# urgent-challenge/urgent2026_challenge_track1

Hardware: AMD Instinct MI355X
Metric: utterances/sec (4 s @ 48 kHz) train step (higher is better)
Workload: dtype bf16

## Files before the change

### include/urse.h

```cpp
#ifndef URSE_H_
#define URSE_H_
#include <stdint.h>

#ifdef __cplusplus
extern "C" {
#endif

#define URSE_OK 0
#define URSE_ERR_INVALID_ARG (-1)
#define URSE_ERR_LAUNCH (-2)
#define URSE_ERR_UNSUPPORTED (-3)
#define URSE_ERR_RUNTIME (-4)

#define URSE_F32 0
#define URSE_BF16 1
#define URSE_F16 2
#define URSE_BF16_ACT_F16 3

#define URSE_WIN_RECT 0
#define URSE_WIN_HANN 1

int urse_version(void);
const char* urse_last_error(void);

#define URSE_KV_NT_BRES 0
#define URSE_KV_NT_RING 1
#define URSE_KV_NT_RING_WIDE 2
#define URSE_KV_NT_128 3
#define URSE_KV_NT_GROUPED_RING 4
#define URSE_KV_NT_GROUPED_128 5
#define URSE_KV_TN_RING 6
#define URSE_KV_TN_RING_T 7
#define URSE_KV_TN_DUAL 8
#define URSE_KV_TN_128 9
#define URSE_KV_TN_GROUPED 10
#define URSE_KV_LSTM_FWD_STREAM 11
#define URSE_KV_LSTM_FWD_WIDE 12
#define URSE_KV_LSTM_FWD_CLUSTER 13
#define URSE_KV_LSTM_FWD_CLUSTER2 14
#define URSE_KV_LSTM_BWD_STREAM16 15
#define URSE_KV_LSTM_BWD_STREAM32 16
#define URSE_KV_LSTM_BWD_CLUSTER 17
#define URSE_KV_LSTM_BWD_SPLIT 18
#define URSE_KV_STFT960 19
#define URSE_KV_STFT_GENERIC 20
#define URSE_KV_ISTFT_GENERIC 21
#define URSE_KV_ISTFT960 22
#define URSE_KV_LSTM_FWD_RW 23
#define URSE_KV_TN_ACT_F16 24
#define URSE_KV_LSTM_FWD_RWX 25
#define URSE_KV_LSTM_BWD_NSPLIT 26
#define URSE_KV_LSTM_FWD_CLUSTERX 27
#define URSE_KV_COUNT 32
int urse_launch_count(int variant);
int urse_launch_counts_reset(void);

int urse_stft_fwd(const float* wav, const int32_t* lens, float* spec, int B, int L, int n_fft, int hop,
                  int window, void* stream);
int urse_istft_fwd(const float* spec, float* wav, int B, int T, int n_fft, int hop, int L_out, int window,
                   void* stream);
int urse_istft_bwd(const float* grad_wav, float* grad_spec, int B, int T, int n_fft, int hop, int L_out,
                   int window, void* stream);

int urse_gemm_nt(const void* A, int64_t lda, const void* B, int64_t ldb, void* C, int64_t ldc, const float* bias,
                 const float* resid, int64_t ldr, int64_t M, int64_t N, int64_t K, int in_dtype, int out_dtype,
                 int act, void* stream);
int urse_gemm_nt_gnstats(const void* A, int64_t lda, const void* B, int64_t ldb, float* C, int64_t ldc, const float* bias,
                         const float* resid, int64_t ldr, int64_t M, int64_t N, int64_t K, int in_dtype, int act,
                         double* stats, int64_t rows_per_group, void* stream);
int urse_gemm_nt_gnbwd(const void* A, int64_t lda, const void* B, int64_t ldb, float* C, int64_t M, int64_t N, int64_t K, int in_dtype,
                       const float* x, const double* stats, const float* gamma, double* sums, float* dgamma, float* dbeta, float* part,
                       int slots, int64_t rows_per_group, float eps, void* stream);
int urse_gemm_nt_grouped(const void* descs, int groups, int max_blocks, int in_dtype, int out_dtype, int act,
                         void* stream);
int urse_gemm_nt_grouped_h(const void* descs, const int64_t* host_descs, int groups, int in_dtype, int out_dtype,
                           int act, void* stream);
int urse_gemm_tn(const void* A, int64_t lda, const void* B, int64_t ldb, float* C, int64_t ldc, float* colsum,
                 int64_t R, int64_t Mo, int64_t No, int64_t shift, int64_t inner, int64_t period,
                 int64_t invalid_step, int64_t perm_h, int dtype, int target_workgroups, void* stream);
int urse_gemm_tn_act_f16_supported(int64_t R, int64_t Mo, int64_t No, int64_t No2, int with_colsum, int64_t inner, int64_t period);
int urse_gemm_tn_dual(const void* A, int64_t lda, const void* B, int64_t ldb, float* C, int64_t ldc, float* colsum,
                      const void* B2, int64_t ldb2, float* C2, int64_t ldc2, int64_t R, int64_t Mo, int64_t No, int64_t No2,
                      int64_t shift, int64_t inner, int64_t period, int64_t invalid_step, int64_t perm_h, int dtype,
                      int target_workgroups, void* stream);
int urse_gemm_tn_grouped(const void* descs, int groups, int max_blocks, int dtype, void* stream);

int urse_groupnorm_fwd(const float* x, const float* gamma, const float* beta, const float* add, void* y, double* stats,
                       int B, int T, int Kg, int W, int N, int Np, int gstride, float eps, int out_dtype, void* y_bf16, void* stream);
int urse_groupnorm_stats(const float* x, double* stats, int B, int T, int Kg, int W, int N, void* stream);
int urse_groupnorm_apply(const float* x, const float* gamma, const float* beta, const float* add, void* y, const double* stats,
                         int B, int T, int Kg, int W, int N, int Np, int gstride, float eps, int out_dtype, void* y_bf16, void* stream);
int urse_groupnorm_bwd(const float* x, const float* dy, const double* stats, const float* gamma, const float* dres,
                       float* dx, float* dgamma, float* dbeta, double* sums, int B, int T, int Kg, int W, int N,
                       int gstride, float eps, void* dx_packed, int ldp, void* stream);
int urse_groupnorm_bwd_apply(const float* x, const float* dy, const double* stats, const double* sums, const float* gamma,
                             const float* dres, float* dx, int B, int T, int Kg, int W, int N, int gstride, float eps, void* dx_packed,
                             int ldp, void* stream);
int urse_pack2d(const void* in, int64_t ldi, int in_dtype, void* out, int64_t ldo, int out_dtype, int rows, int cols,
                int out_rows, int out_cols, int transpose, void* stream);

int urse_pack_segments(const float* in, void* out, const void* segs, int nseg, int blocks_per_seg, int transpose,
                       int out_dtype, void* stream);

int urse_lstm_pack(const float* wih, const float* whh, const float* bih, const float* bhh, void* wih_p, void* wihT_p,
                   float* bias, void* whh_frag, void* whhT_frag, int N, int Np, int H, int Hp, int dtype,
// ... 173 lines not shown
```

### urgent2026_challenge_track1_amd/csrc/gemm.hip

```cpp
#include <stdlib.h>

#include <type_traits>
#include "urse_common.h"

namespace urse {

typedef __bf16 bf16x8_t __attribute__((ext_vector_type(8)));
typedef short short8_t __attribute__((ext_vector_type(8)));
typedef short short4_t __attribute__((ext_vector_type(4)));
typedef float f32x4_t __attribute__((ext_vector_type(4)));

struct GemmDesc {
  const char* A;
  const char* B;
  char* C;
  const float* bias;
  const float* resid;
  long lda, ldb, ldc;
  long M, N, K;
  long ldr;
};

constexpr int BM = 128, BN = 128;
constexpr int SLAB = 64;
// ... 1142 lines not shown
#pragma unroll 1
    for (int h = 0; h < nh; ++h) {
      if constexpr (BH) compute_h(slot + h);
      else compute(slot + h);
      T2ST(4 + h);
    }
    slot ^= 2;
#ifdef T224STAMP
    ++it_;
#endif
  }
  }
  asm volatile("s_waitcnt vmcnt(0)" ::: "memory");

#pragma unroll
  for (int j = 0; j < NT; ++j) {
    const long v = n0 + (wn * NT + j) * 16 + (lane & 15);
    float* dst = nullptr;
    long ld = 0, col = 0;
    if (v < p.No) { dst = p.C; ld = p.ldc; col = v; }
    else if (v >= No8 && v < V) { dst = p.C2; ld = p.ldc2; col = v - No8; }
    else if (v == vones) { dst = p.colsum; ld = 1; col = 0; }
    if (dst == nullptr) continue;
#pragma unroll
    for (int i = 0; i < MT; ++i)
#pragma unroll
      for (int r = 0; r < 4; ++r) {
        const long row = m0 + wm * (MT * 16) + i * 16 + (lane >> 4) * 4 + r;
        atomicAdd(dst + tn_perm(row, p.perm_h) * ld + col, acc[i][j][r]);
      }
  }
}

static void launch_tn_dma(int ntw, int csm, dim3 grid, hipStream_t st, const TnArgs& p, int cvt = 0) {
  if (cvt == 1) { hipLaunchKernelGGL((gemm_tn_dma_kernel<7, 2, 1>), grid, dim3(512), 0, st, p); return; }
#define URSE_TN_L(N_, C_) hipLaunchKernelGGL((gemm_tn_dma_kernel<N_, C_>), grid, dim3(512), 0, st, p)
  if (ntw == 7) { if (csm == 0) URSE_TN_L(7, 0); else if (csm == 1) URSE_TN_L(7, 1); else URSE_TN_L(7, 2); }
  else { if (csm == 0) URSE_TN_L(8, 0); else if (csm == 1) URSE_TN_L(8, 1); else URSE_TN_L(8, 2); }
#undef URSE_TN_L
}

struct NtExtra {
  double* gstats;
  long rpg;
  const float* gnb_x;
  const double* gnb_stats;
  const float* gnb_gamma;
  double* gnb_sums;
  float* gnb_part;
  int gnb_slots;
  float gnb_eps;
};

template <typename TO, int NTW, int ACT, int BMX, int WNC, int GNB = 0, typename TI = bf16_t>
__device__ __forceinline__ void gemm_nt_dma_body(const GemmDesc& d, double* gstats = nullptr, long rpg = 0, const NtExtra* xt = nullptr) {
  constexpr int BNX = 16 * NTW * WNC, NWV = BMX / 64 * WNC, NTHR = NWV * 64;
  constexpr int BNR = WNC == 2 ? 256 : 16 * NTW * WNC;
  constexpr int NST = NWV == 8 ? URSE_NT_NST : 3, STAGE = (BMX + BNR) * 64, BOFF = BMX * 64;
  constexpr int AI = (BMX / 16 + NWV - 1) / NWV;
  constexpr int BI = (BNR / 16 + NWV - 1) / NWV;
  constexpr int DPW = AI + BI;
  static_assert(AI * NWV * 16 == BMX, "A image blocks divide evenly over the waves");
  __shared__ __attribute__((aligned(1024))) char lds[NST * STAGE + 1024];
  const int tn = (int)((d.N + BNX - 1) / BNX), tm = (int)((d.M + BMX - 1) / BMX);
  if ((int)blockIdx.x >= tm * tn) return;
  const int bid = xcd_remap(blockIdx.x, tm * tn);
  const int tile_m = bid / tn, tile_n = bid - tile_m * tn;
  const long m0 = (long)tile_m * BMX, n0 = (long)tile_n * BNX;
  const int tid = threadIdx.x, lane = tid & 63;
  const int w = __builtin_amdgcn_readfirstlane(tid >> 6), wm = w / WNC, wn = w % WNC;
  const int nk = (int)(d.K / 32);
  const char* zsrc = reinterpret_cast<const char*>(g_tn_zero_page) + lane * 16;
  const int srow = lane >> 2, schunk = (lane & 3) ^ ((lane >> 3) & 3);
  const int lc = lane & 15, lr = lane >> 4;
  const int foff = lc * 64 + ((lr ^ ((lc >> 1) & 3)) << 4);

  const char* pa[AI];
  const char* pb[BI];
  bool aok[AI], bok[BI];
#pragma unroll
  for (int j = 0; j < AI; ++j) {
    const int rowl = 16 * (AI * w + j) + srow;
    aok[j] = rowl < BMX && m0 + rowl < d.M;
    pa[j] = d.A + ((m0 + rowl) * d.lda) * 2 + schunk * 16;
  }
#pragma unroll
  for (int j = 0; j < BI; ++j) {
    const int rowl = 16 * (BI * w + j) + srow;
    bok[j] = rowl < BNX && n0 + rowl < d.N;
    pb[j] = d.B + ((n0 + rowl) * d.ldb) * 2 + schunk * 16;
  }
  auto issue = [&](int kt, int slot) {
    char* sbase = lds + slot * STAGE;
    const bool kin = kt < nk;
#pragma unroll
    for (int j = 0; j < AI; ++j) glds16((kin && aok[j]) ? pa[j] + (long)kt * 64 : zsrc, sbase + (AI * w + j) * 1024);
#pragma unroll
    for (int j = 0; j < BI; ++j) {
      const int blk = BI * w + j;
      glds16((kin && bok[j]) ? pb[j] + (long)kt * 64 : zsrc, blk < BNR / 16 ? sbase + BOFF + blk * 1024 : lds + NST * STAGE);
    }
  };
#pragma unroll
  for (int s = 0; s < NST - 1; ++s) issue(s, s);

  constexpr int OS = sizeof(TO);
  f32x4_t bv[NTW];
#pragma unroll
  for (int j = 0; j < NTW; ++j) {
    const long col = n0 + (wn * NTW + j) * 16 + lr * 4;
#pragma unroll
    for (int r = 0; r < 4; ++r) bv[j][r] = (d.bias && col + r < d.N) ? d.bias[col + r] : 0.f;
  }
  f32x4_t acc[4][NTW];
#pragma unroll
  for (int i = 0; i < 4; ++i)
#pragma unroll
    for (int j = 0; j < NTW; ++j) acc[i][j] = f32x4_t{0.f, 0.f, 0.f, 0.f};

  int slot = 0;
  for (int kt = 0; kt < nk; ++kt) {
    if ((NST - 2) * DPW == 12) asm volatile("s_waitcnt vmcnt(12)" ::: "memory");
    else if ((NST - 2) * DPW == 10) asm volatile("s_waitcnt vmcnt(10)" ::: "memory");
    else if ((NST - 2) * DPW == 8) asm volatile("s_waitcnt vmcnt(8)" ::: "memory");
    else asm volatile("s_waitcnt vmcnt(6)" ::: "memory");
    static_assert((NST - 2) * DPW == 12 || (NST - 2) * DPW == 10 || (NST - 2) * DPW == 8 || (NST - 2) * DPW == 6, "wait count");
    __builtin_amdgcn_s_barrier();
    int nslot = slot + NST - 1;
    if (nslot >= NST) nslot -= NST;
    issue(kt + NST - 1, nslot);
    const char* As = lds + slot * STAGE + wm * 4096 + foff;
    const char* Bs = lds + slot * STAGE + BOFF + wn * NTW * 1024 + foff;
    short8_t a[4];
#pragma unroll
    for (int i = 0; i < 4; ++i) a[i] = *reinterpret_cast<const short8_t*>(As + i * 1024);
    short8_t b[NTW];
#pragma unroll
    for (int j = 0; j < NTW; ++j) b[j] = *reinterpret_cast<const short8_t*>(Bs + j * 1024);
#if URSE_NT_SETPRIO
    __builtin_amdgcn_s_setprio(1);
#endif
#pragma unroll
    for (int j = 0; j < NTW; ++j)
#pragma unroll
      for (int i = 0; i < 4; ++i) acc[i][j] = Frag<TI>::mma(b[j], a[i], acc[i][j]);
#if URSE_NT_SETPRIO
    __builtin_amdgcn_s_setprio(0);
#endif
    if (++slot == NST) slot = 0;
  }
  asm volatile("s_waitcnt vmcnt(0)" ::: "memory");
  __syncthreads();
#ifdef NABL_NO_EPI
  if (acc[0][0][0] == 123.456f) d.C[0] = 1;
  return;
#endif

  constexpr int CP = BNX * OS + 16;
  constexpr int RPP = (BMX * CP <= NST * STAGE) ? BMX : ((BMX / 2 * CP <= NST * STAGE) ? BMX / 2 : BMX / 4);
  static_assert(RPP * CP <= NST * STAGE && RPP >= 64, "staging does not fit");
  constexpr int EPC = 16 / OS;
  constexpr int CPR = BNX / EPC;
  TO* C = reinterpret_cast<TO*>(d.C);
  constexpr bool C2K = __is_same(TI, f16_t) && OS == 2 && ACT == 1;
  bf16_t* C2 = (C2K && d.resid) ? reinterpret_cast<bf16_t*>(const_cast<float*>(d.resid)) : nullptr;
  const bool vec_ok = ((d.ldc * OS) % 16 == 0) && ((reinterpret_cast<uintptr_t>(d.C) % 16) == 0) &&
                      (!d.resid || ACT == 2 || (((d.ldr * 4) % 16 == 0) && (reinterpret_cast<uintptr_t>(d.resid) % 16) == 0)) &&
                      (!C2 || (d.ldr * 2) % 16 == 0);
  float gsa = 0.f, gqa = 0.f, gsb = 0.f, gqb = 0.f;
  const bool gst = OS == 4 && gstats != nullptr;
  const long gidx = gst ? m0 / rpg : 0, gbound = gst ? (gidx + 1) * rpg : 0;
  float gnb_m[2] = {0.f, 0.f}, gnb_r[2] = {0.f, 0.f}, gnb_ga[4] = {0.f, 0.f, 0.f, 0.f}, gnb_dg[4] = {0.f, 0.f, 0.f, 0.f}, gnb_db[4] = {0.f, 0.f, 0.f, 0.f};
  long gnb_g0 = 0, gnb_bound = 0;
  constexpr int GXI = GNB ? (RPP + NTHR / CPR - 1) / (NTHR / CPR) : 1, GXA = GXI < 8 ? GXI : 8;
  float4 gnb_xpre[GXI];
  if constexpr (GNB) {
    gnb_g0 = m0 / xt->rpg;
    gnb_bound = (gnb_g0 + 1) * xt->rpg;
    const double cnt = (double)xt->rpg * (double)d.N;
#pragma unroll
    for (int q = 0; q < 2; ++q) {
      const long g = gnb_g0 + q;
      if (g * xt->rpg < d.M) {
        const double mu = xt->gnb_stats[g * 2] / cnt;
        double var = xt->gnb_stats[g * 2 + 1] / cnt - mu * mu;
        if (var < 0.0) var = 0.0;
        gnb_m[q] = (float)mu;
        gnb_r[q] = (float)(1.0 / sqrt(var + (double)xt->gnb_eps));
      }
    }
    const int chf = tid % (BNX / (16 / OS));
    const long col = n0 + chf * (16 / OS);
#pragma unroll
    for (int q = 0; q < 4; ++q) gnb_ga[q] = (col + q < d.N) ? xt->gnb_gamma[col + q] : 0.f;
  }
#pragma unroll 1
  for (int pass = 0; pass < BMX / RPP; ++pass) {
    if (pass > 0) __syncthreads();
    if constexpr (GNB) {
      constexpr int SLOTS = NTHR / CPR, XI = (RPP + SLOTS - 1) / SLOTS;
      const int slot = tid / CPR, chf = tid - slot * CPR;
      const long col = n0 + chf * EPC;
      static_assert(XI == GXI, "prefetch array");
#pragma unroll
      for (int i = 0; i < GXA; ++i) {
        const int lr_ = slot + i * SLOTS;
        const long row = m0 + pass * RPP + lr_;
        const bool ok = slot < SLOTS && col < d.N && lr_ < RPP && row < d.M;
        gnb_xpre[i] = ok ? *reinterpret_cast<const float4*>(xt->gnb_x + row * d.ldc + col) : make_float4(0.f, 0.f, 0.f, 0.f);
      }
    }
    if ((wm * 64) / RPP == pass) {
      const int rbase = (wm * 64) % RPP;
// ... 145 lines not shown
      pb[tid] = make_float4(gnb_db[0], gnb_db[1], gnb_db[2], gnb_db[3]);
    }
    __syncthreads();
    if (tid < 4) {
      double t = 0.0;
      for (int i = 0; i < NWV; ++i) t += red[i * 4 + tid];
      const long g = gnb_g0 + (tid >> 1);
      if ((tid < 2 || gnb_bound < m0 + BMX) && g * xt->rpg < d.M) atomicAdd(xt->gnb_sums + g * 2 + (tid & 1), t);
    }
    if (tid >= 64 && tid < 64 + CPR) {
      const int chf = tid - 64;
      const long col = n0 + chf * EPC;
      if (col < d.N) {
        float4 sg = make_float4(0.f, 0.f, 0.f, 0.f), sb = sg;
        for (int i = 0; i < SLOTS; ++i) {
          const float4 a = pg[i * CPR + chf], bq = pb[i * CPR + chf];
          sg.x += a.x; sg.y += a.y; sg.z += a.z; sg.w += a.w;
          sb.x += bq.x; sb.y += bq.y; sb.z += bq.z; sb.w += bq.w;
        }
        float* part = xt->gnb_part + (long)(blockIdx.x % xt->gnb_slots) * 2 * d.N;
        const float vg[4] = {sg.x, sg.y, sg.z, sg.w}, vb[4] = {sb.x, sb.y, sb.z, sb.w};
        for (int q = 0; q < 4 && col + q < d.N; ++q) {
          atomicAdd(part + col + q, vg[q]);
          atomicAdd(part + d.N + col + q, vb[q]);
        }
      }
    }
    return;
  }
  if (gst) {
    __syncthreads();
    double* red = reinterpret_cast<double*>(lds);
    const double r0 = wave_sum_d((double)gsa), r1 = wave_sum_d((double)gqa), r2 = wave_sum_d((double)gsb), r3 = wave_sum_d((double)gqb);
    if (lane == 0) { red[w * 4] = r0; red[w * 4 + 1] = r1; red[w * 4 + 2] = r2; red[w * 4 + 3] = r3; }
    __syncthreads();
    if (tid < 4) {
      double t = 0.0;
      for (int i = 0; i < NWV; ++i) t += red[i * 4 + tid];
      const long g = gidx + (tid >> 1);
      if (tid < 2 || gbound < m0 + BMX) {
        if (g * rpg < d.M) atomicAdd(gstats + g * 2 + (tid & 1), t);
      }
    }
  }
}

template <typename TO, int NTW, int ACT, int BMX, int WNC = 2, typename TI = bf16_t>
__global__ void __launch_bounds__(BMX / 64 * WNC * 64) gemm_nt_dma_kernel(GemmDesc d, NtExtra x) {
  gemm_nt_dma_body<TO, NTW, ACT, BMX, WNC, 0, TI>(d, x.gstats, x.rpg);
}

__global__ void __launch_bounds__(512) gemm_nt_dma_gnb_kernel(GemmDesc d, NtExtra x) {
  gemm_nt_dma_body<float, 7, 0, 256, 2, 1>(d, nullptr, 0, &x);
}

__global__ void gnb_fold_kernel(const float* __restrict__ part, int slots, int N, float* __restrict__ dgamma, float* __restrict__ dbeta) {
  const int c = blockIdx.x * blockDim.x + threadIdx.x;
  if (c >= N) return;
  float a = 0.f, b = 0.f;
  for (int s = 0; s < slots; ++s) { a += part[(long)s * 2 * N + c]; b += part[(long)s * 2 * N + N + c]; }
  dgamma[c] += a;
  dbeta[c] += b;
}

template <typename TO, int ACT, typename TI = bf16_t>
__global__ void __launch_bounds__(512) gemm_nt_dma_grouped_kernel(const GemmDesc* __restrict__ descs) {
  const GemmDesc d = descs[blockIdx.y];
  gemm_nt_dma_body<TO, 7, ACT, 256, 2, 0, TI>(d);
}

template <int ACT, typename TI = bf16_t>
__global__ void __launch_bounds__(512) gemm_nt_bres_kernel(GemmDesc d, int wg_per_slice) {
  constexpr int BMX = 256, NTW = 7, BNX = 224, NST = 3, STAGE = BMX * 64, KSTEPS = 7, BRES = KSTEPS * 14 * 1024;
  __shared__ __attribute__((aligned(1024))) char lds[BRES + NST * STAGE];
  char* ring = lds + BRES;
  const int tm = (int)((d.M + BMX - 1) / BMX);
  const int tile_n = blockIdx.x / wg_per_slice, part = blockIdx.x - tile_n * wg_per_slice;
  const long n0 = (long)tile_n * BNX;
  const int tid = threadIdx.x, lane = tid & 63;
  const int w = __builtin_amdgcn_readfirstlane(tid >> 6), wm = w >> 1, wn = w & 1;
  const int nk = (int)(d.K / 32);
  const char* zsrc = reinterpret_cast<const char*>(g_tn_zero_page) + lane * 16;
  const int srow = lane >> 2, schunk = (lane & 3) ^ ((lane >> 3) & 3);
  const int lc = lane & 15, lr = lane >> 4;
  const int foff = lc * 64 + ((lr ^ ((lc >> 1) & 3)) << 4);
  for (int blk = w; blk < nk * 14; blk += 8) {
    const int kt = blk / 14, b = blk - kt * 14;
    const long row = n0 + b * 16 + srow;
    glds16(row < d.N ? d.B + (row * d.ldb) * 2 + schunk * 16 + (long)kt * 64 : zsrc, lds + blk * 1024);
  }
  f32x4_t bv[NTW];
#pragma unroll
  for (int j = 0; j < NTW; ++j) {
    const long col = n0 + (wn * NTW + j) * 16 + lr * 4;
#pragma unroll
    for (int r = 0; r < 4; ++r) bv[j][r] = (d.bias && col + r < d.N) ? d.bias[col + r] : 0.f;
  }
  bf16_t* C = reinterpret_cast<bf16_t*>(d.C);
  auto tile_src = [&](int mt, const char* (&pa)[2], bool (&aok)[2]) __attribute__((always_inline)) {
#pragma unroll
    for (int j = 0; j < 2; ++j) {
      const long row = (long)mt * BMX + 16 * (2 * w + j) + srow;
      aok[j] = mt < tm && row < d.M;
      pa[j] = d.A + (row * d.lda) * 2 + schunk * 16;
    }
  };
// ... 295 lines not shown
    long rpp = (M + parts - 1) / parts;
    rpp = (rpp + WR_ROWS - 1) / WR_ROWS * WR_ROWS;
    dim3 grid((unsigned)(tn * parts));
    hipStream_t st = (hipStream_t)stream;
    note_launch(URSE_KV_NT_BRES);
    if (act == 0) hipLaunchKernelGGL(gemm_nt_wreg_kernel<0>, grid, dim3(448), 0, st, d, parts, rpp);
    else hipLaunchKernelGGL(gemm_nt_wreg_kernel<1>, grid, dim3(448), 0, st, d, parts, rpp);
    URSE_CHECK_LAUNCH("urse_gemm_nt");
    return URSE_OK;
  }
#endif
  if (bres_mode && in16 && out16 && !no_dma && M >= 8192 && N >= g_nt_bres_min_n && K % 32 == 0 &&
      K >= 96 && K <= 224 && !resid && act != 2 && (ldc * 2) % 16 == 0 && ((uintptr_t)C % 16) == 0) {
    const int tn = (int)((N + 223) / 224);
    int per = g_nt_bres_wgs / tn;
    if (per < 1) per = 1;
    dim3 grid((unsigned)(tn * per));
    hipStream_t st = (hipStream_t)stream;
    note_launch(URSE_KV_NT_BRES);
    if (f16) {
      if (act == 0) hipLaunchKernelGGL((gemm_nt_bres_kernel<0, f16_t>), grid, dim3(512), 0, st, d, per);
      else hipLaunchKernelGGL((gemm_nt_bres_kernel<1, f16_t>), grid, dim3(512), 0, st, d, per);
    } else if (act == 0) hipLaunchKernelGGL(gemm_nt_bres_kernel<0>, grid, dim3(512), 0, st, d, per);
    else hipLaunchKernelGGL(gemm_nt_bres_kernel<1>, grid, dim3(512), 0, st, d, per);
    URSE_CHECK_LAUNCH("urse_gemm_nt");
    return URSE_OK;
  }
  if (in16 && !no_dma && M >= 2048 && N >= 160 && K % 32 == 0 && K >= 96 && !(f16 && act == 2)) {
    const long pad7 = (N + 223) / 224 * 224, pad8 = (N + 255) / 256 * 256;
    int ntw = pad7 <= pad8 ? 7 : 8;
    if (const char* e = getenv("URSE_NT_NTW")) ntw = atoi(e) == 8 ? 8 : 7;
    int bmx = 256;
    if (const char* e = getenv("URSE_NT_BMX")) bmx = atoi(e) == 128 ? 128 : 256;
    int wide = g_nt_wide_default && K <= g_nt_wide_maxk && N >= 1792 && out_dtype == URSE_BF16 && (N + 447) / 448 * 448 <= pad7 + 64;
    if (const char* e = getenv("URSE_NT_WIDE")) wide = atoi(e) != 0 && N >= 448;
    if (f16) { wide = 0; bmx = 256; }
    const long tl = wide ? ((M + 127) / 128) * ((N + 447) / 448) : ((M + bmx - 1) / bmx) * ((N + 32L * ntw - 1) / (32L * ntw));
    URSE_CHECK_ARG(tl < (1L << 31), "urse_gemm_nt: too many tiles");
    dim3 grid((unsigned)tl);
    hipStream_t st = (hipStream_t)stream;
    if (gstats && out_dtype == URSE_F32 && act != 2 && !wide && rpg >= bmx) {
      xtra.gstats = gstats;
      xtra.rpg = rpg;
      if (fused) *fused = 1;
    }
#define URSE_NT_DMA(TO_, NTW_, ACT_, BMX_) \
  hipLaunchKernelGGL((gemm_nt_dma_kernel<TO_, NTW_, ACT_, BMX_>), grid, dim3(BMX_ * 2), 0, st, d, xtra)
#define URSE_NT_DMA_W(TO_, ACT_) \
  hipLaunchKernelGGL((gemm_nt_dma_kernel<TO_, 7, ACT_, 128, 4>), grid, dim3(512), 0, st, d, xtra)
#define URSE_NT_DMA_B(TO_, NTW_, ACT_) do { if (wide) URSE_NT_DMA_W(TO_, ACT_); else if (bmx == 128) URSE_NT_DMA(TO_, NTW_, ACT_, 128); else URSE_NT_DMA(TO_, NTW_, ACT_, 256); } while (0)
#define URSE_NT_DMA_ACT(TO_, NTW_) \
  do { if (act == 0) URSE_NT_DMA_B(TO_, NTW_, 0); else if (act == 1) URSE_NT_DMA_B(TO_, NTW_, 1); else URSE_NT_DMA_B(TO_, NTW_, 2); } while (0)
    note_launch(wide ? URSE_KV_NT_RING_WIDE : URSE_KV_NT_RING);
    if (f16) {
#define URSE_NT_DMA_H(TO_, NTW_, ACT_) hipLaunchKernelGGL((gemm_nt_dma_kernel<TO_, NTW_, ACT_, 256, 2, f16_t>), grid, dim3(512), 0, st, d, xtra)
#define URSE_NT_DMA_H_ACT(TO_, NTW_) do { if (act == 0) URSE_NT_DMA_H(TO_, NTW_, 0); else URSE_NT_DMA_H(TO_, NTW_, 1); } while (0)
      if (out_dtype == URSE_F16) { if (ntw == 7) URSE_NT_DMA_H_ACT(f16_t, 7); else URSE_NT_DMA_H_ACT(f16_t, 8); }
      else { if (ntw == 7) URSE_NT_DMA_H_ACT(float, 7); else URSE_NT_DMA_H_ACT(float, 8); }
    } else if (out_dtype == URSE_BF16) {
      if (ntw == 7) URSE_NT_DMA_ACT(bf16_t, 7); else URSE_NT_DMA_ACT(bf16_t, 8);
    } else {
      if (ntw == 7) URSE_NT_DMA_ACT(float, 7); else URSE_NT_DMA_ACT(float, 8);
    }
    URSE_CHECK_LAUNCH("urse_gemm_nt");
    return URSE_OK;
  }
  const long blocks = ((M + BM - 1) / BM) * ((N + BN - 1) / BN);
  URSE_CHECK_ARG(blocks < (1L << 31), "urse_gemm_nt: too many tiles");
  note_launch(URSE_KV_NT_128);
  return dispatch_nt(nullptr, d, 1, (int)blocks, in_dtype, out_dtype, act, (hipStream_t)stream);
}

extern "C" int urse_gemm_nt(const void* A, int64_t lda, const void* B, int64_t ldb, void* C, int64_t ldc,
                            const float* bias, const float* resid, int64_t ldr, int64_t M, int64_t N, int64_t K,
                            int in_dtype, int out_dtype, int act, void* stream) {
  return gemm_nt_impl(A, lda, B, ldb, C, ldc, bias, resid, ldr, M, N, K, in_dtype, out_dtype, act, stream, nullptr, 0, nullptr);
}

extern "C" int urse_gemm_nt_gnstats(const void* A, int64_t lda, const void* B, int64_t ldb, float* C, int64_t ldc,
                                    const float* bias, const float* resid, int64_t ldr, int64_t M, int64_t N, int64_t K,
                                    int in_dtype, int act, double* stats, int64_t rows_per_group, void* stream) {
  URSE_CHECK_ARG(stats && rows_per_group > 0 && M % rows_per_group == 0 && ldc == N && N % 4 == 0,
                 "urse_gemm_nt_gnstats: needs whole groups of rows, a dense output and N %% 4 == 0");
  const int groups = (int)(M / rows_per_group);
  (void)hipMemsetAsync(stats, 0, sizeof(double) * 2 * groups, (hipStream_t)stream);
  int fused = 0;
  int rc = gemm_nt_impl(A, lda, B, ldb, C, ldc, bias, resid, ldr, M, N, K, in_dtype, URSE_F32, act, stream, stats, rows_per_group,
                        &fused);
  if (rc || fused) return rc;
  return urse_groupnorm_stats(C, stats, groups, (int)rows_per_group, 1, (int)N, (int)N, stream);
}

extern "C" int urse_gemm_nt_gnbwd(const void* A, int64_t lda, const void* B, int64_t ldb, float* C, int64_t M, int64_t N, int64_t K,
                                  int in_dtype, const float* x, const double* stats, const float* gamma, double* sums, float* dgamma,
                                  float* dbeta, float* part, int slots, int64_t rows_per_group, float eps, void* stream) {
  URSE_CHECK_ARG(A && B && C && x && stats && gamma && sums && dgamma && dbeta && part && slots > 0 && rows_per_group > 0,
                 "urse_gemm_nt_gnbwd: bad argument");
  static const bool no_dma = getenv("URSE_NT_NO_DMA") != nullptr;
  if (no_dma || in_dtype != URSE_BF16 || M < 2048 || N < 160 || N > 224 || N % 4 || K % 32 || K < 96 || rows_per_group < 256 ||
      M % rows_per_group || ((uintptr_t)C % 16) || ((uintptr_t)x % 16)) {
    set_error("urse_gemm_nt_gnbwd: shape M%ld N%ld K%ld not served by the fused kernel", (long)M, (long)N, (long)K);
    return URSE_ERR_UNSUPPORTED;
  }
  GemmDesc d;
  d.A = (const char*)A; d.B = (const char*)B; d.C = (char*)C; d.bias = nullptr; d.resid = nullptr;
  d.lda = lda; d.ldb = ldb; d.ldc = N; d.M = M; d.N = N; d.K = K; d.ldr = 0;
  int rc = check_desc_host(d, 2, "urse_gemm_nt_gnbwd");
  if (rc) return rc;
  hipStream_t st = (hipStream_t)stream;
  const size_t sums_bytes = sizeof(double) * 2 * (size_t)(M / rows_per_group), part_bytes = sizeof(float) * 2 * (size_t)N * slots;
  if (reinterpret_cast<char*>(part) == reinterpret_cast<char*>(sums) + sums_bytes) {
    (void)hipMemsetAsync(sums, 0, sums_bytes + part_bytes, st);
  } else {
    (void)hipMemsetAsync(sums, 0, sums_bytes, st);
    (void)hipMemsetAsync(part, 0, part_bytes, st);
  }
  NtExtra xt{};
  xt.rpg = rows_per_group; xt.gnb_x = x; xt.gnb_stats = stats; xt.gnb_gamma = gamma; xt.gnb_sums = sums; xt.gnb_part = part;
  xt.gnb_slots = slots; xt.gnb_eps = eps;
  const long tl = (M + 255) / 256;
  URSE_CHECK_ARG(tl < (1L << 31), "urse_gemm_nt_gnbwd: too many tiles");
  note_launch(URSE_KV_NT_RING);
  hipLaunchKernelGGL(gemm_nt_dma_gnb_kernel, dim3((unsigned)tl), dim3(512), 0, st, d, xt);
  hipLaunchKernelGGL(gnb_fold_kernel, dim3((unsigned)((N + 255) / 256)), dim3(256), 0, st, part, slots, (int)N, dgamma, dbeta);
  URSE_CHECK_LAUNCH("urse_gemm_nt_gnbwd");
  return URSE_OK;
}

extern "C" int urse_gemm_nt_grouped(const void* descs, int groups, int max_blocks, int in_dtype, int out_dtype,
                                    int act, void* stream) {
  URSE_CHECK_ARG(descs && groups > 0 && max_blocks > 0, "urse_gemm_nt_grouped: bad argument");
  GemmDesc dummy;
  memset(&dummy, 0, sizeof(dummy));
  note_launch(URSE_KV_NT_GROUPED_128);
  return dispatch_nt((const GemmDesc*)descs, dummy, groups, max_blocks, in_dtype, out_dtype, act,
                     (hipStream_t)stream);
}

extern "C" int urse_gemm_nt_grouped_h(const void* descs, const int64_t* host_descs, int groups, int in_dtype,
                                      int out_dtype, int act, void* stream) {
  URSE_CHECK_ARG(descs && host_descs && groups > 0 && groups < 65536, "urse_gemm_nt_grouped_h: bad argument");
  const GemmDesc* hd = reinterpret_cast<const GemmDesc*>(host_descs);
  const bool f16 = in_dtype == URSE_F16;
  const int es = (in_dtype == URSE_BF16 || f16) ? 2 : 4;
  URSE_CHECK_ARG(out_dtype == URSE_F32 || (out_dtype == URSE_BF16 && !f16) || (out_dtype == URSE_F16 && f16),
                 "urse_gemm_nt_grouped_h: output dtype %d with operand dtype %d", out_dtype, in_dtype);
  bool dma = es == 2 && !(f16 && act == 2) && !getenv("URSE_NT_NO_DMA") && !getenv("URSE_NT_GROUPED_NO_DMA");
  long t128 = 0, tdma = 0;
  const char* mm = getenv("URSE_NT_GROUPED_MIN_M");
  const long min_m = mm ? atol(mm) : 1024;
  for (int g = 0; g < groups; ++g) {
    const GemmDesc& d = hd[g];
    if (int rc = check_desc_host(d, es, "urse_gemm_nt_grouped_h")) return rc;
    dma = dma && d.K % 32 == 0 && d.N >= 160 && d.M >= min_m;
    t128 = std::max(t128, ((d.M + BM - 1) / BM) * ((d.N + BN - 1) / BN));
    tdma = std::max(tdma, ((d.M + 255) / 256) * ((d.N + 223) / 224));
  }
  URSE_CHECK_ARG(t128 < (1L << 31), "urse_gemm_nt_grouped_h: too many tiles");
  if (!dma) {
    GemmDesc dummy;
    memset(&dummy, 0, sizeof(dummy));
    note_launch(URSE_KV_NT_GROUPED_128);
    return dispatch_nt((const GemmDesc*)descs, dummy, groups, (int)t128, in_dtype, out_dtype, act, (hipStream_t)stream);
  }
  dim3 grid((unsigned)tdma, (unsigned)groups);
  hipStream_t st = (hipStream_t)stream;
  const GemmDesc* dd = (const GemmDesc*)descs;
#define URSE_NT_G(TO_, ACT_) hipLaunchKernelGGL((gemm_nt_dma_grouped_kernel<TO_, ACT_>), grid, dim3(512), 0, st, dd)
#define URSE_NT_G_ACT(TO_) do { if (act == 0) URSE_NT_G(TO_, 0); else if (act == 1) URSE_NT_G(TO_, 1); else URSE_NT_G(TO_, 2); } while (0)
  note_launch(URSE_KV_NT_GROUPED_RING);
#define URSE_NT_GH(TO_, ACT_) hipLaunchKernelGGL((gemm_nt_dma_grouped_kernel<TO_, ACT_, f16_t>), grid, dim3(512), 0, st, dd)
  if (f16 && out_dtype == URSE_F16) { if (act == 0) URSE_NT_GH(f16_t, 0); else URSE_NT_GH(f16_t, 1); }
  else if (f16) { if (act == 0) URSE_NT_GH(float, 0); else URSE_NT_GH(float, 1); }
  else if (out_dtype == URSE_BF16) URSE_NT_G_ACT(bf16_t);
  else if (out_dtype == URSE_F32) URSE_NT_G_ACT(float);
  else { set_error("urse_gemm_nt_grouped_h: bad output dtype %d", out_dtype); return URSE_ERR_INVALID_ARG; }
// ... 203 lines not shown
```

### urgent2026_challenge_track1_amd/ops.py

```python
import os

import torch

from . import _lib
from ._lib import call, require_cuda, stream_ptr

WIN_RECT, WIN_HANN = 0, 1
F32, BF16, F16 = 0, 1, 2
BF16_ACT_F16 = 3
HALF_TYPES = (torch.bfloat16, torch.float16)


def bwd_dtype(dtype):
    return torch.bfloat16 if dtype == torch.float16 else dtype

_timing = None


def enable_timing(names):
    global _timing
    _timing = {n: [] for n in names}


def disable_timing():
    global _timing
    t, _timing = _timing, None
    return t


def timed_call(tname, name, *args):
    if _timing is not None and tname in _timing:
        a, b = torch.cuda.Event(enable_timing=True), torch.cuda.Event(enable_timing=True)
        a.record()
        call(name, *args)
        b.record()
        _timing[tname].append((a, b))
    else:
        call(name, *args)


KERNEL_VARIANTS = ("nt_bres", "nt_ring", "nt_ring_wide", "nt_128", "nt_grouped_ring", "nt_grouped_128", "tn_ring", "tn_ring_t",
                   "tn_dual", "tn_128", "tn_grouped", "lstm_fwd_stream", "lstm_fwd_wide", "lstm_fwd_cluster",
                   "lstm_fwd_cluster2", "lstm_bwd_stream16", "lstm_bwd_stream32", "lstm_bwd_cluster", "lstm_bwd_split",
                   "stft960", "stft_generic", "istft_generic", "istft960", "lstm_fwd_rw", "tn_act_f16", "lstm_fwd_rwx", "lstm_bwd_nsplit",
                   "lstm_fwd_clusterx", "_unused28")


_PAGEABLE_UPLOADS = os.environ.get("URSE_PAGEABLE_UPLOADS", "0") == "1"


def upload(host_tensor, device, cached=False):
    if torch.device(device).type != "cuda":
        return host_tensor
    if _PAGEABLE_UPLOADS:
        return host_tensor.to(device)
    out = host_tensor.contiguous().pin_memory().to(device, non_blocking=True)
    if cached:
        ev = torch.cuda.Event()
        ev.record(torch.cuda.current_stream(device))
        ev.synchronize()
    return out


def launch_counts(reset=False):
    lib = _lib.load()
    out = {n: lib.urse_launch_count(i) for i, n in enumerate(KERNEL_VARIANTS)}
    if reset:
        lib.urse_launch_counts_reset()
    return out


def _f32c(t):
    return t.contiguous().float() if (t.dtype != torch.float32 or not t.is_contiguous()) else t


def stft_forward(wav, n_fft, hop, window=WIN_HANN, lens=None):
    require_cuda(wav)
    wav = _f32c(wav)
    B, L = wav.shape
    T, Fb = L // hop + 1, n_fft // 2 + 1
    spec = torch.empty(B, T, Fb, 2, device=wav.device, dtype=torch.float32)
    if lens is not None:
        if lens.device.type == "cpu":
            lens = upload(lens.to(torch.int32), wav.device)
        else:
            lens = lens.to(device=wav.device, dtype=torch.int32).contiguous()
    timed_call("stft_fwd", "stft_fwd", wav, lens, spec, B, L, n_fft, hop, window, stream_ptr())
    return torch.view_as_complex(spec)


class _ISTFT(torch.autograd.Function):
    @staticmethod
    def forward(ctx, spec_ri, n_fft, hop, length, window):
        B, T, Fb, _ = spec_ri.shape
        wav = torch.empty(B, length, device=spec_ri.device, dtype=torch.float32)
        call("istft_fwd", spec_ri, wav, B, T, n_fft, hop, length, window, stream_ptr())
        ctx.cfg = (B, T, Fb, n_fft, hop, length, window)
        return wav
# ... 912 lines not shown
```

Before: 252.3.

## Add 64-deep K stages to the 256x224 NT GEMM for the GroupNorm-backward dgrad

Adds a K-depth-64 variant of the NT ring GEMM body for the 256x224 tile. A uses a three-slot ring and B a two-slot ring, with a new 128-byte-row swizzle and half-step fragment reads. By default it runs only for the GroupNorm-backward dgrad GEMM when K >= 192; the FC site stays at depth 32 unless overridden by an environment variable. The aim is to halve the number of barriers and wait points per K and raise MFMA work per sync, at the cost of more LDS per block, which may reduce occupancy, and an odd-K tail handled by per-chunk bounds.

```diff
diff --git a/include/urse.h b/include/urse.h
--- a/include/urse.h
+++ b/include/urse.h
@@ -51,6 +51,7 @@
 #define URSE_KV_LSTM_FWD_RWX 25
 #define URSE_KV_LSTM_BWD_NSPLIT 26
 #define URSE_KV_LSTM_FWD_CLUSTERX 27
+#define URSE_KV_NT_RING_K64 29
 #define URSE_KV_COUNT 32
 int urse_launch_count(int variant);
 int urse_launch_counts_reset(void);
diff --git a/urgent2026_challenge_track1_amd/csrc/gemm.hip b/urgent2026_challenge_track1_amd/csrc/gemm.hip
--- a/urgent2026_challenge_track1_amd/csrc/gemm.hip
+++ b/urgent2026_challenge_track1_amd/csrc/gemm.hip
@@ -1218,7 +1218,7 @@
   float gnb_eps;
 };
 
-template <typename TO, int NTW, int ACT, int BMX, int WNC, int GNB = 0, typename TI = bf16_t>
+template <typename TO, int NTW, int ACT, int BMX, int WNC, int GNB = 0, typename TI = bf16_t, int KD = 32>
 __device__ __forceinline__ void gemm_nt_dma_body(const GemmDesc& d, double* gstats = nullptr, long rpg = 0, const NtExtra* xt = nullptr) {
   constexpr int BNX = 16 * NTW * WNC, NWV = BMX / 64 * WNC, NTHR = NWV * 64;
   constexpr int BNR = WNC == 2 ? 256 : 16 * NTW * WNC;
@@ -1227,7 +1227,10 @@
   constexpr int BI = (BNR / 16 + NWV - 1) / NWV;
   constexpr int DPW = AI + BI;
   static_assert(AI * NWV * 16 == BMX, "A image blocks divide evenly over the waves");
-  __shared__ __attribute__((aligned(1024))) char lds[NST * STAGE + 1024];
+  constexpr int K64A = 256 * 128, K64B = BNX * 128;
+  constexpr int RING = KD == 64 ? 3 * K64A + 2 * K64B : NST * STAGE;
+  static_assert(KD == 32 || (KD == 64 && BMX == 256 && WNC == 2 && NTW == 7 && sizeof(TI) == 2), "64-deep stages: the 256 x 224 tile only");
+  __shared__ __attribute__((aligned(1024))) char lds[RING + 1024];
   const int tn = (int)((d.N + BNX - 1) / BNX), tm = (int)((d.M + BMX - 1) / BMX);
   if ((int)blockIdx.x >= tm * tn) return;
   const int bid = xcd_remap(blockIdx.x, tm * tn);
@@ -1235,85 +1238,151 @@
   const long m0 = (long)tile_m * BMX, n0 = (long)tile_n * BNX;
   const int tid = threadIdx.x, lane = tid & 63;
   const int w = __builtin_amdgcn_readfirstlane(tid >> 6), wm = w / WNC, wn = w % WNC;
-  const int nk = (int)(d.K / 32);
   const char* zsrc = reinterpret_cast<const char*>(g_tn_zero_page) + lane * 16;
-  const int srow = lane >> 2, schunk = (lane & 3) ^ ((lane >> 3) & 3);
   const int lc = lane & 15, lr = lane >> 4;
-  const int foff = lc * 64 + ((lr ^ ((lc >> 1) & 3)) << 4);
-
-  const char* pa[AI];
-  const char* pb[BI];
-  bool aok[AI], bok[BI];
-#pragma unroll
-  for (int j = 0; j < AI; ++j) {
-    const int rowl = 16 * (AI * w + j) + srow;
-    aok[j] = rowl < BMX && m0 + rowl < d.M;
-    pa[j] = d.A + ((m0 + rowl) * d.lda) * 2 + schunk * 16;
-  }
-#pragma unroll
-  for (int j = 0; j < BI; ++j) {
-    const int rowl = 16 * (BI * w + j) + srow;
-    bok[j] = rowl < BNX && n0 + rowl < d.N;
-    pb[j] = d.B + ((n0 + rowl) * d.ldb) * 2 + schunk * 16;
-  }
-  auto issue = [&](int kt, int slot) {
-    char* sbase = lds + slot * STAGE;
-    const bool kin = kt < nk;
-#pragma unroll
-    for (int j = 0; j < AI; ++j) glds16((kin && aok[j]) ? pa[j] + (long)kt * 64 : zsrc, sbase + (AI * w + j) * 1024);
-#pragma unroll
-    for (int j = 0; j < BI; ++j) {
-      const int blk = BI * w + j;
-      glds16((kin && bok[j]) ? pb[j] + (long)kt * 64 : zsrc, blk < BNR / 16 ? sbase + BOFF + blk * 1024 : lds + NST * STAGE);
-    }
-  };
-#pragma unroll
-  for (int s = 0; s < NST - 1; ++s) issue(s, s);
-
   constexpr int OS = sizeof(TO);
   f32x4_t bv[NTW];
-#pragma unroll
-  for (int j = 0; j < NTW; ++j) {
-    const long col = n0 + (wn * NTW + j) * 16 + lr * 4;
-#pragma unroll
-    for (int r = 0; r < 4; ++r) bv[j][r] = (d.bias && col + r < d.N) ? d.bias[col + r] : 0.f;
-  }
   f32x4_t acc[4][NTW];
-#pragma unroll
-  for (int i = 0; i < 4; ++i)
-#pragma unroll
-    for (int j = 0; j < NTW; ++j) acc[i][j] = f32x4_t{0.f, 0.f, 0.f, 0.f};
-
-  int slot = 0;
-  for (int kt = 0; kt < nk; ++kt) {
-    if ((NST - 2) * DPW == 12) asm volatile("s_waitcnt vmcnt(12)" ::: "memory");
-    else if ((NST - 2) * DPW == 10) asm volatile("s_waitcnt vmcnt(10)" ::: "memory");
-    else if ((NST - 2) * DPW == 8) asm volatile("s_waitcnt vmcnt(8)" ::: "memory");
-    else asm volatile("s_waitcnt vmcnt(6)" ::: "memory");
-    static_assert((NST - 2) * DPW == 12 || (NST - 2) * DPW == 10 || (NST - 2) * DPW == 8 || (NST - 2) * DPW == 6, "wait count");
-    __builtin_amdgcn_s_barrier();
-    int nslot = slot + NST - 1;
-    if (nslot >= NST) nslot -= NST;
-    issue(kt + NST - 1, nslot);
-    const char* As = lds + slot * STAGE + wm * 4096 + foff;
-    const char* Bs = lds + slot * STAGE + BOFF + wn * NTW * 1024 + foff;
-    short8_t a[4];
-#pragma unroll
-    for (int i = 0; i < 4; ++i) a[i] = *reinterpret_cast<const short8_t*>(As + i * 1024);
-    short8_t b[NTW];
-#pragma unroll
-    for (int j = 0; j < NTW; ++j) b[j] = *reinterpret_cast<const short8_t*>(Bs + j * 1024);
+  auto init_acc = [&]() {
+#pragma unroll
+    for (int j = 0; j < NTW; ++j) {
+      const long col = n0 + (wn * NTW + j) * 16 + lr * 4;
+#pragma unroll
+      for (int r = 0; r < 4; ++r) bv[j][r] = (d.bias && col + r < d.N) ? d.bias[col + r] : 0.f;
+    }
+#pragma unroll
+    for (int i = 0; i < 4; ++i)
+#pragma unroll
+      for (int j = 0; j < NTW; ++j) acc[i][j] = f32x4_t{0.f, 0.f, 0.f, 0.f};
+
+  };
+  if constexpr (KD == 64) {
+    constexpr int BBASE = 3 * K64A, NBB = BNX / 8;
+    const int nk = (int)((d.K + 32) / 64);
+    const int nkf = (int)(d.K / 64);
+    const int r8 = lane >> 3;
+    const int foff = lc * 128 + ((lr ^ ((lc >> 1) & 7)) << 4);
+    const char* pa[4];
+    const char* pb[4];
+    bool aok[4], bok[4];
+    const int sc0 = (lane & 7) ^ (r8 >> 1);
+    const int nke = sc0 < 4 ? nk : nkf, nko = sc0 < 4 ? nkf : nk;
+#pragma unroll
+    for (int j = 0; j < 4; ++j) {
+      const int rowl = 32 * w + 8 * j + r8, sc = sc0 ^ ((j & 1) << 2);
+      aok[j] = m0 + rowl < d.M;
+      pa[j] = d.A + ((m0 + rowl) * d.lda) * 2 + sc * 16;
+      bok[j] = rowl < BNX && n0 + rowl < d.N;
+      pb[j] = d.B + ((n0 + rowl) * d.ldb) * 2 + sc * 16;
+    }
+    auto issue_a = [&](int kt, int slot) {
+      char* sbase = lds + slot * K64A + w * 4096;
+#pragma unroll
+      for (int j = 0; j < 4; ++j) glds16((kt < ((j & 1) ? nko : nke) && aok[j]) ? pa[j] + (long)kt * 128 : zsrc, sbase + j * 1024);
+    };
+    auto issue_b = [&](int kt, int slot) {
+      char* sbase = lds + BBASE + slot * K64B;
+#pragma unroll
+      for (int j = 0; j < 4; ++j) {
+        const int blk = 4 * w + j;
+        glds16((kt < ((j & 1) ? nko : nke) && bok[j]) ? pb[j] + (long)kt * 128 : zsrc, blk < NBB ? sbase + blk * 1024 : lds + RING);
+      }
+    };
+    issue_a(0, 0);
+    issue_b(0, 0);
+    issue_a(1, 1);
+    init_acc();
+    int sa = 0, sb = 0;
+    for (int kt = 0; kt < nk; ++kt) {
+      asm volatile("s_waitcnt vmcnt(4)" ::: "memory");
+      __builtin_amdgcn_s_barrier();
+      issue_b(kt + 1, sb ^ 1);
+      issue_a(kt + 2, sa >= 1 ? sa - 1 : 2);
+      const char* As = lds + sa * K64A + wm * 8192;
+      const char* Bs = lds + BBASE + sb * K64B + wn * NTW * 2048;
+#pragma unroll
+      for (int h = 0; h < 2; ++h) {
+        const int fo = foff ^ (h << 6);
+        short8_t a[4];
+#pragma unroll
+        for (int i = 0; i < 4; ++i) a[i] = *reinterpret_cast<const short8_t*>(As + i * 2048 + fo);
+        short8_t b[NTW];
+#pragma unroll
+        for (int j = 0; j < NTW; ++j) b[j] = *reinterpret_cast<const short8_t*>(Bs + j * 2048 + fo);
+#pragma unroll
+        for (int j = 0; j < NTW; ++j)
+#pragma unroll
+          for (int i = 0; i < 4; ++i) acc[i][j] = Frag<TI>::mma(b[j], a[i], acc[i][j]);
+      }
+      if (++sa == 3) sa = 0;
+      sb ^= 1;
+    }
+  } else {
+    const int nk = (int)(d.K / 32);
+    const int srow = lane >> 2, schunk = (lane & 3) ^ ((lane >> 3) & 3);
+    const int foff = lc * 64 + ((lr ^ ((lc >> 1) & 3)) << 4);
+
+    const char* pa[AI];
+    const char* pb[BI];
+    bool aok[AI], bok[BI];
+#pragma unroll
+    for (int j = 0; j < AI; ++j) {
+      const int rowl = 16 * (AI * w + j) + srow;
+      aok[j] = rowl < BMX && m0 + rowl < d.M;
+      pa[j] = d.A + ((m0 + rowl) * d.lda) * 2 + schunk * 16;
+    }
+#pragma unroll
+    for (int j = 0; j < BI; ++j) {
+      const int rowl = 16 * (BI * w + j) + srow;
+      bok[j] = rowl < BNX && n0 + rowl < d.N;
+      pb[j] = d.B + ((n0 + rowl) * d.ldb) * 2 + schunk * 16;
+    }
+    auto issue = [&](int kt, int slot) {
+      char* sbase = lds + slot * STAGE;
+      const bool kin = kt < nk;
+#pragma unroll
+      for (int j = 0; j < AI; ++j) glds16((kin && aok[j]) ? pa[j] + (long)kt * 64 : zsrc, sbase + (AI * w + j) * 1024);
+#pragma unroll
+      for (int j = 0; j < BI; ++j) {
+        const int blk = BI * w + j;
+        glds16((kin && bok[j]) ? pb[j] + (long)kt * 64 : zsrc, blk < BNR / 16 ? sbase + BOFF + blk * 1024 : lds + NST * STAGE);
+      }
+    };
+#pragma unroll
+    for (int s = 0; s < NST - 1; ++s) issue(s, s);
+
+    init_acc();
+    int slot = 0;
+    for (int kt = 0; kt < nk; ++kt) {
+      if ((NST - 2) * DPW == 12) asm volatile("s_waitcnt vmcnt(12)" ::: "memory");
+      else if ((NST - 2) * DPW == 10) asm volatile("s_waitcnt vmcnt(10)" ::: "memory");
+      else if ((NST - 2) * DPW == 8) asm volatile("s_waitcnt vmcnt(8)" ::: "memory");
+      else asm volatile("s_waitcnt vmcnt(6)" ::: "memory");
+      static_assert((NST - 2) * DPW == 12 || (NST - 2) * DPW == 10 || (NST - 2) * DPW == 8 || (NST - 2) * DPW == 6, "wait count");
+      __builtin_amdgcn_s_barrier();
+      int nslot = slot + NST - 1;
+      if (nslot >= NST) nslot -= NST;
+      issue(kt + NST - 1, nslot);
+      const char* As = lds + slot * STAGE + wm * 4096 + foff;
+      const char* Bs = lds + slot * STAGE + BOFF + wn * NTW * 1024 + foff;
+      short8_t a[4];
+#pragma unroll
+      for (int i = 0; i < 4; ++i) a[i] = *reinterpret_cast<const short8_t*>(As + i * 1024);
+      short8_t b[NTW];
+#pragma unroll
+      for (int j = 0; j < NTW; ++j) b[j] = *reinterpret_cast<const short8_t*>(Bs + j * 1024);
 #if URSE_NT_SETPRIO
-    __builtin_amdgcn_s_setprio(1);
-#endif
-#pragma unroll
-    for (int j = 0; j < NTW; ++j)
-#pragma unroll
-      for (int i = 0; i < 4; ++i) acc[i][j] = Frag<TI>::mma(b[j], a[i], acc[i][j]);
+      __builtin_amdgcn_s_setprio(1);
+#endif
+#pragma unroll
+      for (int j = 0; j < NTW; ++j)
+#pragma unroll
+        for (int i = 0; i < 4; ++i) acc[i][j] = Frag<TI>::mma(b[j], a[i], acc[i][j]);
 #if URSE_NT_SETPRIO
-    __builtin_amdgcn_s_setprio(0);
-#endif
-    if (++slot == NST) slot = 0;
+      __builtin_amdgcn_s_setprio(0);
+#endif
+      if (++slot == NST) slot = 0;
+    }
   }
   asm volatile("s_waitcnt vmcnt(0)" ::: "memory");
   __syncthreads();
@@ -1323,8 +1392,8 @@
 #endif
 
   constexpr int CP = BNX * OS + 16;
-  constexpr int RPP = (BMX * CP <= NST * STAGE) ? BMX : ((BMX / 2 * CP <= NST * STAGE) ? BMX / 2 : BMX / 4);
-  static_assert(RPP * CP <= NST * STAGE && RPP >= 64, "staging does not fit");
+  constexpr int RPP = (BMX * CP <= RING) ? BMX : ((BMX / 2 * CP <= RING) ? BMX / 2 : BMX / 4);
+  static_assert(RPP * CP <= RING && RPP >= 64, "staging does not fit");
   constexpr int EPC = 16 / OS;
   constexpr int CPR = BNX / EPC;
   TO* C = reinterpret_cast<TO*>(d.C);
@@ -1576,6 +1645,24 @@
 
 __global__ void __launch_bounds__(512) gemm_nt_dma_gnb_kernel(GemmDesc d, NtExtra x) {
   gemm_nt_dma_body<float, 7, 0, 256, 2, 1>(d, nullptr, 0, &x);
+}
+
+template <typename TO, int NTW, int ACT>
+__global__ void __launch_bounds__(512) gemm_nt_dma_k64_kernel(GemmDesc d, NtExtra x) {
+  gemm_nt_dma_body<TO, NTW, ACT, 256, 2, 0, bf16_t, 64>(d, x.gstats, x.rpg);
+}
+__global__ void __launch_bounds__(512) gemm_nt_dma_gnb_k64_kernel(GemmDesc d, NtExtra x) {
+  gemm_nt_dma_body<float, 7, 0, 256, 2, 1, bf16_t, 64>(d, nullptr, 0, &x);
+}
+enum { NT_SITE_DGRAD = 0, NT_SITE_FC = 1 };
+constexpr int NT_KDEPTH_DEFAULT[2] = {64, 32};
+static int nt_kdepth(int site, long K) {
+  if (const char* e = getenv("URSE_NT_KDEPTH")) {
+    if (!strcmp(e, "dgrad")) return site == NT_SITE_DGRAD ? 64 : 32;
+    if (!strcmp(e, "fc")) return site == NT_SITE_FC ? 64 : 32;
+    return atoi(e) == 64 ? 64 : 32;
+  }
+  return K >= 192 ? NT_KDEPTH_DEFAULT[site] : 32;
 }
 
 __global__ void gnb_fold_kernel(const float* __restrict__ part, int slots, int N, float* __restrict__ dgamma, float* __restrict__ dbeta) {
@@ -1977,7 +2064,10 @@
 #define URSE_NT_DMA_ACT(TO_, NTW_) \
   do { if (act == 0) URSE_NT_DMA_B(TO_, NTW_, 0); else if (act == 1) URSE_NT_DMA_B(TO_, NTW_, 1); else URSE_NT_DMA_B(TO_, NTW_, 2); } while (0)
     note_launch(wide ? URSE_KV_NT_RING_WIDE : URSE_KV_NT_RING);
-    if (f16) {
+    if (in_dtype == URSE_BF16 && out_dtype == URSE_F32 && act == 0 && ntw == 7 && bmx == 256 && !wide && nt_kdepth(NT_SITE_FC, K) == 64) {
+      note_launch(URSE_KV_NT_RING_K64);
+      hipLaunchKernelGGL((gemm_nt_dma_k64_kernel<float, 7, 0>), grid, dim3(512), 0, st, d, xtra);
+    } else if (f16) {
 #define URSE_NT_DMA_H(TO_, NTW_, ACT_) hipLaunchKernelGGL((gemm_nt_dma_kernel<TO_, NTW_, ACT_, 256, 2, f16_t>), grid, dim3(512), 0, st, d, xtra)
 #define URSE_NT_DMA_H_ACT(TO_, NTW_) do { if (act == 0) URSE_NT_DMA_H(TO_, NTW_, 0); else URSE_NT_DMA_H(TO_, NTW_, 1); } while (0)
       if (out_dtype == URSE_F16) { if (ntw == 7) URSE_NT_DMA_H_ACT(f16_t, 7); else URSE_NT_DMA_H_ACT(f16_t, 8); }
@@ -2046,7 +2136,12 @@
   const long tl = (M + 255) / 256;
   URSE_CHECK_ARG(tl < (1L << 31), "urse_gemm_nt_gnbwd: too many tiles");
   note_launch(URSE_KV_NT_RING);
-  hipLaunchKernelGGL(gemm_nt_dma_gnb_kernel, dim3((unsigned)tl), dim3(512), 0, st, d, xt);
+  if (nt_kdepth(NT_SITE_DGRAD, K) == 64) {
+    note_launch(URSE_KV_NT_RING_K64);
+    hipLaunchKernelGGL(gemm_nt_dma_gnb_k64_kernel, dim3((unsigned)tl), dim3(512), 0, st, d, xt);
+  } else {
+    hipLaunchKernelGGL(gemm_nt_dma_gnb_kernel, dim3((unsigned)tl), dim3(512), 0, st, d, xt);
+  }
   hipLaunchKernelGGL(gnb_fold_kernel, dim3((unsigned)((N + 255) / 256)), dim3(256), 0, st, part, slots, (int)N, dgamma, dbeta);
   URSE_CHECK_LAUNCH("urse_gemm_nt_gnbwd");
   return URSE_OK;
diff --git a/urgent2026_challenge_track1_amd/ops.py b/urgent2026_challenge_track1_amd/ops.py
--- a/urgent2026_challenge_track1_amd/ops.py
+++ b/urgent2026_challenge_track1_amd/ops.py
@@ -43,7 +43,7 @@
                    "tn_dual", "tn_128", "tn_grouped", "lstm_fwd_stream", "lstm_fwd_wide", "lstm_fwd_cluster",
                    "lstm_fwd_cluster2", "lstm_bwd_stream16", "lstm_bwd_stream32", "lstm_bwd_cluster", "lstm_bwd_split",
                    "stft960", "stft_generic", "istft_generic", "istft960", "lstm_fwd_rw", "tn_act_f16", "lstm_fwd_rwx", "lstm_bwd_nsplit",
-                   "lstm_fwd_clusterx", "_unused28")
+                   "lstm_fwd_clusterx", "_unused28", "nt_ring_k64")
 
 
 _PAGEABLE_UPLOADS = os.environ.get("URSE_PAGEABLE_UPLOADS", "0") == "1"
```

Result: no change. 253.2 (median of 2 runs) (+0.3%).
